# mnlevy1981/MOM6

Hardware: AMD Instinct MI355X
Metric: simulated-years/day (SYPD) of the split-RK2 dynamical core + tracer advection + ALE remap (higher is better)
Workload: dtype f64

## Files before the change

### mom6_amd/csrc/barotropic.hip

```cpp
#include "common.hpp"
#include "cr_math.hpp"

#include <algorithm>
#include <cmath>
#include <cstdlib>
#include <string>
#include <vector>

namespace {

constexpr double SUBROUNDOFF = 1e-30;

using m6::cr::cr_pow;

template <class F> __global__ void __launch_bounds__(256) range2d_kernel(int i0, int i1, int j0, int j1, F f) {
  const int i = i0 + blockIdx.x * 64 + threadIdx.x, j = j0 + blockIdx.y * 4 + threadIdx.y;
  if (i <= i1 && j <= j1) f(i, j);
}
template <class F> void launch2d(hipStream_t st, int i0, int i1, int j0, int j1, F f) {
  if (i1 < i0 || j1 < j0) return;
  dim3 grid((i1 - i0 + 64) / 64, (j1 - j0 + 4) / 4), block(64, 4);
  hipLaunchKernelGGL(range2d_kernel<F>, grid, block, 0, st, i0, i1, j0, j1, f);
}

// ... 152 lines not shown
#pragma unroll
  for (int k = 1; k < NKMAX; k++) if (k < nz) tot = tot + v[k];
  const double Ihat = mask / (tot + h_neglect);
  double *__restrict__ dst = fr + f2;
#pragma unroll
  for (int k = 0; k < NKMAX; k++) { if (k < nz) *dst = v[k] * Ihat; dst += fstr; }
}

template <int DIR>
__global__ void __launch_bounds__(256)
bt_accel_layer_kernel(m6::GridDev g, Work w, const double *__restrict__ pbce, double *__restrict__ accel, double accel_underflow) {
  const int i = (DIR ? g.isc : g.isc - 1) + blockIdx.x * 64 + threadIdx.x;
  const int j = (DIR ? g.jsc - 1 : g.jsc) + blockIdx.y * 4 + threadIdx.y;
  if (i > g.iec || j > g.jec) return;
  const long f2 = DIR ? g.v2(i, j) : g.u2(i, j);
  const long fstr = DIR ? (long)g.nih * (g.njh + 1) : (long)(g.nih + 1) * g.njh;
  const long hm = g.h2(i, j), hp = DIR ? g.h2(i, j + 1) : g.h2(i + 1, j), hstr = (long)g.nih * g.njh;
  const double abt = DIR ? w.v_accel_bt[f2] : w.u_accel_bt[f2];
  const double gp = DIR ? w.gtot_S[hp] : w.gtot_W[hp], gm = DIR ? w.gtot_N[hm] : w.gtot_E[hm];
  const double ep = w.e_anom[hp], em = w.e_anom[hm];
  const double Id = DIR ? g.IdyCv[f2] : g.IdxCu[f2];
  for (int k = 0; k < g.nk; k++) {
    double a = (abt - ((pbce[hp + hstr * k] - gp) * ep - (pbce[hm + hstr * k] - gm) * em) * Id);
    if (fabs(a) < accel_underflow) a = 0.0;
    accel[f2 + fstr * k] = a;
  }
}

__global__ void __launch_bounds__(256)
bt_eta_pred_kernel(m6::GridDev g, Work w, Par p, int i0, int i1, int j0, int j1, double wt_accel2) {
  const int i = i0 + blockIdx.x * 64 + threadIdx.x, j = j0 + blockIdx.y * 4 + threadIdx.y;
  if (i > i1 || j > j1) return;
  const long n = g.h2(i, j);
  double ep;
  if (p.project_velocity) {
    ep = w.eta[n];
  } else {
    ep = (w.eta[n] + w.eta_src[n]) + (p.dtbt * g.IareaT[n]) *
        ((w.uhbtp[g.u2(i - 1, j)] - w.uhbtp[g.u2(i, j)]) + (w.vhbtp[g.v2(i, j - 1)] - w.vhbtp[g.v2(i, j)]));
    w.eta_pred[n] = ep;
  }
  if (p.find_etaav && i >= g.isc && i <= g.iec && j >= g.jsc && j <= g.jec) w.eta_sum[n] = w.eta_sum[n] + wt_accel2 * ep;
}

__global__ void __launch_bounds__(256)
bt_eta_kernel(m6::GridDev g, Work w, Par p, int i0, int i1, int j0, int j1, double wt_eta) {
  const int i = i0 + blockIdx.x * 64 + threadIdx.x, j = j0 + blockIdx.y * 4 + threadIdx.y;
  if (i > i1 || j > j1) return;
  const long n = g.h2(i, j);
  const double e = (w.eta[n] + w.eta_src[n]) + (p.dtbt * g.IareaT[n]) *
      ((w.uhbt[g.u2(i - 1, j)] - w.uhbt[g.u2(i, j)]) + (w.vhbt[g.v2(i, j - 1)] - w.vhbt[g.v2(i, j)]));
  w.eta[n] = e;
  w.eta_wtd[n] = w.eta_wtd[n] + e * wt_eta;
}

__device__ __forceinline__ double eta_pf_at(const Work &w, const Par &p, long n, double wt_end) {
  return p.interp_eta_PF ? (w.eta_PF_1[n] + wt_end * w.d_eta_PF[n]) : w.eta_PF[n];
}

__global__ void __launch_bounds__(256)
bt_vbt_kernel(m6::GridDev g, Work w, Par p, int i0, int i1, int j0, int j1, double wt_accel, double wt_trans, double wt_end,
              double *__restrict__ vbt_sum, double *__restrict__ vhbt_sum) {
  const int i = i0 + blockIdx.x * 64 + threadIdx.x, J = j0 + blockIdx.y * 4 + threadIdx.y;
  if (i > i1 || J > j1) return;
  const int j = J;
  const long n = g.v2(i, J);
  if (w.obc_v && w.obc_v[n]) return;
  const double Cor_v = -1.0 * ((w.amer[g.u2(i - 1, j)] * w.ubt[g.u2(i - 1, j)] + w.cmer[g.u2(i, j + 1)] * w.ubt[g.u2(i, j + 1)]) +
                               (w.bmer[g.u2(i, j)] * w.ubt[g.u2(i, j)] + w.dmer[g.u2(i - 1, j + 1)] * w.ubt[g.u2(i - 1, j + 1)])) -
                       w.Cor_ref_v[n];
  const long hs = g.h2(i, j), hn = g.h2(i, j + 1);
  const double *epb = p.project_velocity ? w.eta : w.eta_pred;
  const double PFv = ((epb[hs] - eta_pf_at(w, p, hs, wt_end)) * w.gtot_N[hs] -
                      (epb[hn] - eta_pf_at(w, p, hn, wt_end)) * w.gtot_S[hn]) * p.dgeo_de * g.IdyCv[n];
  const double vel_prev = w.vbt[n];
  double vb = w.bt_rem_v[n] * (vel_prev + p.dtbt * ((w.BT_force_v[n] + Cor_v) + PFv));
  if (fabs(vb) < p.vel_underflow) vb = 0.0;
  const double vtrans = p.trans_wt1 * vb + p.trans_wt2 * vel_prev;
  w.vbt[n] = vb;
  w.v_accel_bt[n] = w.v_accel_bt[n] + wt_accel * (Cor_v + PFv);
  const double vh0 = w.vhbt0[n];
  double vh, vhp;
  if (p.use_BT_cont) { vh = find_uhbt(vtrans, w.BV, n) + vh0; vhp = find_uhbt(vb, w.BV, n) + vh0; }
  else { const double D = w.Datv[n]; vh = D * vtrans + vh0; vhp = D * vb + vh0; }
  w.vhbt[n] = vh; w.vhbtp[n] = vhp;
  if (i >= g.isc && i <= g.iec && J >= g.jsc - 1 && J <= g.jec) {
    vbt_sum[n] = vbt_sum[n] + wt_trans * vtrans;
    vhbt_sum[n] = vhbt_sum[n] + wt_trans * vh;
  }
}

__global__ void __launch_bounds__(256)
bt_ubt_kernel(m6::GridDev g, Work w, Par p, int i0, int i1, int j0, int j1, double wt_accel, double wt_trans, double wt_end,
              double *__restrict__ ubt_sum, double *__restrict__ uhbt_sum) {
  const int I = i0 + blockIdx.x * 64 + threadIdx.x, j = j0 + blockIdx.y * 4 + threadIdx.y;
  if (I > i1 || j > j1) return;
  const int i = I;
  const long n = g.u2(I, j);
  if (w.obc_u && w.obc_u[n]) return;
  const double Cor_u = ((w.azon[n] * w.vbt[g.v2(i + 1, j)] + w.czon[n] * w.vbt[g.v2(i, j - 1)]) +
                        (w.bzon[n] * w.vbt[g.v2(i, j)] + w.dzon[n] * w.vbt[g.v2(i + 1, j - 1)])) - w.Cor_ref_u[n];
  const long hw = g.h2(i, j), he = g.h2(i + 1, j);
  const double *epb = p.project_velocity ? w.eta : w.eta_pred;
  const double PFu = ((epb[hw] - eta_pf_at(w, p, hw, wt_end)) * w.gtot_E[hw] -
                      (epb[he] - eta_pf_at(w, p, he, wt_end)) * w.gtot_W[he]) * p.dgeo_de * g.IdxCu[n];
  const double vel_prev = w.ubt[n];
// ... 1032 lines not shown
  const int halo = ievf - ie, s_is = is - halo, s_ie = ie + halo, s_js = js - halo, s_je = je + halo;
  const double g_prime1 = g.g_Earth, H_to_Z = g.H_to_Z, Z_ref = cs->Z_ref;
  for (int d = 0; d < 2; d++) {
    if (!(d ? apply_v_OBCs : apply_u_OBCs)) continue;
    double *o_outer = d ? w.ob_vbt_outer : w.ob_ubt_outer, *o_dZ = d ? w.ob_dZ_v : w.ob_dZ_u,
           *o_Cg = d ? w.ob_Cg_v : w.ob_Cg_u, *o_SSH = d ? w.ob_SSH_v : w.ob_SSH_u;
    const int32_t *code = d ? w.obc_v : w.obc_u;
    launch2d(s, d ? s_is : s_is - 1, s_ie, d ? s_js - 1 : s_js, s_je, [=] __device__(int i, int j) {
      const long f = d ? g.v2(i, j) : g.u2(i, j);
      const int c = code[f];
      if (!c || (c & OB_SPEC)) return;
      {
        const long cc = (c & OB_PLUS) ? g.h2(i, j) : (d ? g.h2(i, j + 1) : g.h2(i + 1, j));
        const double dZ = g.bathyT[cc] + H_to_Z * w.eta[cc];
        o_dZ[f] = dZ;
        o_Cg[f] = sqrt(1.0 * g_prime1 * dZ);
      }
    });
    if (d ? obc->Flather_v_BCs_exist_globally : obc->Flather_u_BCs_exist_globally)
      for (int n = 0; n < obc->number_of_segments; n++) {
        const mom6hip_obc_segment_t &S = obc->segment[n];
        if (!((d ? S.is_N_or_S : S.is_E_or_W) && S.Flather)) continue;
        M6_REQUIRE(S.normal_vel_bt && S.SSH, "btstep: segment %d is a Flather segment: normal_vel_bt and SSH are required", n + 1);
        const int a0 = d ? S.isd : S.IsdB, a1 = d ? S.ied : S.IedB, b0 = d ? S.JsdB : S.jsd, b1 = d ? S.JedB : S.jed;
        const long na = a1 - a0 + 1, nb = b1 - b0 + 1;
        const double *nv = st.in(S.normal_vel_bt, (size_t)na * nb * 8), *ssh = st.in(S.SSH, (size_t)na * nb * 8);
        M6_REQUIRE(!st.failed() && nv && ssh, "btstep: staging failed");
        launch2d(s, a0, a1, b0, b1, [=] __device__(int a, int b) {
          const long f = d ? g.v2(a, b) : g.u2(a, b), q = (a - a0) + na * (b - b0);
          o_outer[f] = nv[q];
          o_SSH[f] = ssh[q] + Z_ref;
        });
      }
  }
  if (int rc = pass2d(ctx, {{w.ob_ubt_outer, PU}, {w.ob_vbt_outer, PV}, {w.ob_uhbt, PU}, {w.ob_vhbt, PV}, {w.ob_SSH_u, PUs}, {w.ob_SSH_v, PVs},
                     {w.ob_dZ_u, PUs}, {w.ob_dZ_v, PVs}, {w.ob_Cg_u, PUs}, {w.ob_Cg_v, PVs}})) return rc;
  return 0;
}

void bt_step_ranges(BtCall &bt) {
  const m6::GridDev &g = bt.g;
  const int is = g.isc, ie = g.iec, js = g.jsc, je = g.jec, isvf = bt.isvf, ievf = bt.ievf, jsvf = bt.jsvf, jevf = bt.jevf;
  const int stencil = bt.stencil, nt = bt.nt; std::vector<StepRange> &rng = bt.rng;
  rng.assign(nt + 1, StepRange{});
  int isv = is, iev = ie, jsv = js, jev = je;
  for (int n = 1; n <= nt; n++) {
    bool pf = false;
    if ((iev - stencil < ie) || (jev - stencil < je)) { pf = true; isv = isvf; iev = ievf; jsv = jsvf; jev = jevf; }
    else { isv += stencil; iev -= stencil; jsv += stencil; jev -= stencil; }
    rng[n] = {isv, iev, jsv, jev, pf};
  }
}

void bt_run_steps(BtCall &bt, hipStream_t st, int n0, int n1) {
  mom6hip_ctx_t *ctx = bt.ctx; const mom6hip_barotropic_cs_t *cs = bt.cs; const m6::GridDev &g = bt.g; const Sizes &sz = bt.sz; const Work &w = bt.w;
  const Par &p = bt.p; const CsDev &c = bt.c; const int is = g.isc, ie = g.iec, js = g.jsc, je = g.jec;
  const bool nonlin_update = bt.nonlin_update, apply_OBCs = bt.apply_OBCs, apply_u_OBCs = bt.apply_u_OBCs, apply_v_OBCs = bt.apply_v_OBCs;
  const std::vector<StepRange> &rng = bt.rng;
  const std::vector<double> &wt_vel = bt.wt_vel, &wt_eta = bt.wt_eta, &wt_trans = bt.wt_trans, &wt_accel = bt.wt_accel, &wt_accel2 = bt.wt_accel2;
  double *duhbtav = bt.duhbtav, *dvhbtav = bt.dvhbtav;
  for (int n = n0; n <= n1; n++) {
    const int isv = rng[n].isv, iev = rng[n].iev, jsv = rng[n].jsv, jev = rng[n].jev;
    const double wt_end = n * p.Instep;
    if (nonlin_update && (n > 1) && ((n - 1) % cs->Nonlin_cont_update_period == 0)) {
      find_face_areas(st, g, w.Datu, w.Datv, w.eta, 0.0, 1 + iev - ie);
      if (!p.project_velocity) {
        launch2d(st, isv - 2, iev + 1, jsv - 1, jev + 1, [=] __device__(int I, int j) {
          const long q = g.u2(I, j);
          w.uhbtp[q] = w.Datu[q] * w.ubt[q] + w.uhbt0[q];
        });
        launch2d(st, isv - 1, iev + 1, jsv - 2, jev + 1, [=] __device__(int i, int J) {
          const long q = g.v2(i, J);
          w.vhbtp[q] = w.Datv[q] * w.vbt[q] + w.vhbt0[q];
        });
      }
    }
    hipLaunchKernelGGL(bt_eta_pred_kernel, grid2d(isv - 1, iev + 1, jsv - 1, jev + 1), dim3(64, 4), 0, st, g, w, p, isv - 1, iev + 1,
                       jsv - 1, jev + 1, wt_accel2[n]);
    const bool v_first = ((n + ctx->host.first_direction) % 2) == 1;
    if (apply_OBCs) {
      (void)hipMemcpyAsync(w.ubt_old, w.ubt, sz.u2, hipMemcpyDeviceToDevice, st);
      (void)hipMemcpyAsync(w.vbt_old, w.vbt, sz.v2, hipMemcpyDeviceToDevice, st);
    }
    for (int ps = 0; ps < 2; ps++) {
      const bool do_v = (ps == 0) ? v_first : !v_first;
      if (do_v) {
        const int i0 = v_first ? isv - 1 : isv, i1 = v_first ? iev + 1 : iev;
        hipLaunchKernelGGL(bt_vbt_kernel, grid2d(i0, i1, jsv - 1, jev), dim3(64, 4), 0, st, g, w, p, i0, i1, jsv - 1, jev, wt_accel[n],
                           wt_trans[n], wt_end, c.vbtav, dvhbtav);
      } else {
        const int j0 = v_first ? jsv : jsv - 1, j1 = v_first ? jev : jev + 1;
        hipLaunchKernelGGL(bt_ubt_kernel, grid2d(isv - 1, iev, j0, j1), dim3(64, 4), 0, st, g, w, p, isv - 1, iev, j0, j1, wt_accel[n],
                           wt_trans[n], wt_end, c.ubtav, duhbtav);
      }
    }
    if (apply_OBCs) {
      const int halo = iev - ie;
      if (apply_u_OBCs)
        hipLaunchKernelGGL(bt_obc_kernel<0>, grid2d(is - halo - 1, ie + halo, js - halo, je + halo), dim3(64, 4), 0, st, g, w, p, is - halo - 1,
                           ie + halo, js - halo, je + halo, cs->bebt, wt_trans[n], wt_vel[n], c.ubtav, duhbtav);
      if (apply_v_OBCs)
        hipLaunchKernelGGL(bt_obc_kernel<1>, grid2d(is - halo, ie + halo, js - halo - 1, je + halo), dim3(64, 4), 0, st, g, w, p, is - halo,
                           ie + halo, js - halo - 1, je + halo, cs->bebt, wt_trans[n], wt_vel[n], c.vbtav, dvhbtav);
    }
    hipLaunchKernelGGL(bt_eta_kernel, grid2d(isv, iev, jsv, jev), dim3(64, 4), 0, st, g, w, p, isv, iev, jsv, jev, wt_eta[n]);
  }
}

int bt_pass_steps(BtCall &bt) {
  const Work &w = bt.w;
  return pass2d(bt.ctx, {{w.eta, PH}, {w.ubt, PU}, {w.vbt, PV}, {w.uhbtp, PU}, {w.vhbtp, PV}});
}

int bt_run_loop(BtCall &bt, hipStream_t st, int n0, int n1) {
  for (int n = n0; n <= n1; n++) {
    if (bt.rng[n].pass_first) { if (int rc = bt_pass_steps(bt)) return rc; }
    bt_run_steps(bt, st, n, n);
  }
  return 0;
}

std::string bt_graph_key(const BtCall &bt) {
  const mom6hip_barotropic_cs_t *cs = bt.cs; const CsDev &c = bt.c;
  std::string base_key;
  auto add = [&](const void *q, size_t nbytes) { base_key.append((const char *)q, nbytes); };
  add(&bt.w, sizeof(bt.w)); add(&bt.p, sizeof(bt.p)); add(&bt.nt, sizeof(bt.nt)); add(&bt.ctx->host.first_direction, sizeof(int32_t));
  { const double ob_key[3] = {bt.apply_u_OBCs ? 1.0 : 0.0, bt.apply_v_OBCs ? 1.0 : 0.0, cs->bebt}; add(ob_key, sizeof(ob_key)); }
  { const int32_t nl[2] = {bt.nonlin_update ? 1 : 0, cs->Nonlin_cont_update_period}; add(nl, sizeof(nl)); }
  add(&c.ubtav, sizeof(double *)); add(&c.vbtav, sizeof(double *)); add(&bt.duhbtav, sizeof(double *)); add(&bt.dvhbtav, sizeof(double *));
  for (const std::vector<double> *wt : {&bt.wt_vel, &bt.wt_eta, &bt.wt_trans, &bt.wt_accel, &bt.wt_accel2})
    add(wt->data(), sizeof(double) * wt->size());
  return base_key;
}

int bt_graph_of(BtCall &bt, const std::string &base_key, int n0, int n1, bool with_passes, hipGraphExec_t *out) {
  mom6hip_ctx_t *ctx = bt.ctx;
  std::string key = base_key;
  key.append((const char *)&n0, sizeof(int)); key.append((const char *)&n1, sizeof(int)); key.push_back(with_passes ? 1 : 0);
  for (auto &e : ctx->bt_graphs) if (e.first == key) { *out = (hipGraphExec_t)e.second; return 0; }
  if (!ctx->cap_stream) M6_HIP(hipStreamCreateWithFlags(&ctx->cap_stream, hipStreamNonBlocking));
  hipStream_t saved = ctx->stream;
  ctx->stream = ctx->cap_stream;
  hipError_t e0 = hipStreamBeginCapture(ctx->cap_stream, hipStreamCaptureModeRelaxed);
  int rc = 1;
  if (e0 == hipSuccess) {
    if (with_passes) rc = bt_run_loop(bt, ctx->cap_stream, n0, n1);
    else { bt_run_steps(bt, ctx->cap_stream, n0, n1); rc = 0; }
  }
  hipGraph_t graph = nullptr;
  hipError_t e1 = (e0 == hipSuccess) ? hipStreamEndCapture(ctx->cap_stream, &graph) : e0;
  ctx->stream = saved;
  M6_REQUIRE(rc == 0 && e1 == hipSuccess && graph, "btstep: capturing the barotropic subcycle as a hipGraph failed (%s)",
             hipGetErrorString(e1));
  { size_t nn = 0; if (hipGraphGetNodes(graph, nullptr, &nn) == hipSuccess) ctx->bt_graph_nodes_last = (long)nn; }
  hipGraphExec_t exec = nullptr;
  hipError_t e2 = hipGraphInstantiate(&exec, graph, nullptr, nullptr, 0);
  (void)hipGraphDestroy(graph);
  M6_REQUIRE(e2 == hipSuccess && exec, "btstep: hipGraphInstantiate failed (%s)", hipGetErrorString(e2));
  if (ctx->bt_graphs.size() >= 256) {
    (void)hipGraphExecDestroy((hipGraphExec_t)ctx->bt_graphs.front().second);
    ctx->bt_graphs.erase(ctx->bt_graphs.begin());
  }
  ctx->bt_graphs.push_back({key, (void *)exec});
  ctx->bt_graph_captures++;
  *out = exec;
  return 0;
}

int bt_segments(const BtCall &bt) {
  int nseg = 0;
  for (int n = 1; n <= bt.nt; n++) if (n == 1 || bt.rng[n].pass_first) nseg++;
  return nseg;
}

int bt_subcycle(BtCall &bt) {
  mom6hip_ctx_t *ctx = bt.ctx; hipStream_t s = bt.s; const int nt = bt.nt; const std::vector<StepRange> &rng = bt.rng;
  static const bool graph_off = getenv("MOM6HIP_BT_GRAPH") && atoi(getenv("MOM6HIP_BT_GRAPH")) == 0;
  if (graph_off || (m6::multi_tile(ctx) && bt_segments(bt) > 100)) {
    if (int rc = bt_run_loop(bt, s, 1, nt)) return rc;
  } else if (m6::multi_tile(ctx)) {
    const std::string base_key = bt_graph_key(bt);
    int n0 = 1;
    while (n0 <= nt) {
      int n1 = n0;
      while (n1 + 1 <= nt && !rng[n1 + 1].pass_first) n1++;
      if (rng[n0].pass_first) { if (int rc = bt_pass_steps(bt)) return rc; }
      hipGraphExec_t exec = nullptr;
      if (int rc = bt_graph_of(bt, base_key, n0, n1, false, &exec)) return rc;
      M6_HIP(hipGraphLaunch(exec, s));
      ctx->bt_graph_launches++;
      n0 = n1 + 1;
    }
  } else {
    hipGraphExec_t exec = nullptr;
    if (int rc = bt_graph_of(bt, bt_graph_key(bt), 1, nt, true, &exec)) return rc;
    m6::KTimer kt(ctx, MOM6HIP_KT_BT_SUBCYCLE);
    M6_HIP(hipGraphLaunch(exec, s));
    ctx->bt_graph_launches++;
  }
  M6_HIP(hipGetLastError());
  return 0;
}

int bt_epilogue(BtCall &bt) {
  mom6hip_ctx_t *ctx = bt.ctx; const m6::GridDev &g = bt.g; const Work &w = bt.w; const Par &p = bt.p; const CsDev &c = bt.c; hipStream_t s = bt.s;
  const int is = g.isc, ie = g.iec, js = g.jsc, je = g.jec;
  const bool interp = bt.interp, find_etaav = bt.find_etaav, apply_OBCs = bt.apply_OBCs, apply_u_OBCs = bt.apply_u_OBCs,
             apply_v_OBCs = bt.apply_v_OBCs;
  const double dt = bt.dt, accel_underflow = bt.accel_underflow; const double *deta_in = bt.deta_in, *dpb = bt.dpb;
  double *dalu = bt.dalu, *dalv = bt.dalv, *deta_out = bt.deta_out, *duhbtav = bt.duhbtav, *dvhbtav = bt.dvhbtav, *detaav = bt.detaav;
  const double dgeo_de = p.dgeo_de;
  launch2d(s, is, ie, js, je, [=] __device__(int i, int j) {
    const long n = g.h2(i, j);
    double ea;
    if (interp) ea = dgeo_de * (0.5 * (w.eta[n] + deta_in[n]) - (w.eta_PF_1[n] + 0.5 * w.d_eta_PF[n]));
    else ea = dgeo_de * (0.5 * (w.eta[n] + deta_in[n]) - w.eta_PF[n]);
    w.e_anom[n] = ea;
    if (find_etaav) detaav[n] = w.eta_sum[n] * 1.0;
    deta_out[n] = w.eta_wtd[n] * 1.0;
  });
  for (int d = 0; d < 2 && apply_OBCs; d++) {
    if (!(d ? apply_v_OBCs : apply_u_OBCs)) continue;
    const int32_t *code = d ? w.obc_v : w.obc_u;
    launch2d(s, d ? is : is - 1, ie, d ? js - 1 : js, je, [=] __device__(int i, int j) {
      const int cde = code[d ? g.v2(i, j) : g.u2(i, j)];
      const long c0 = g.h2(i, j), c1 = d ? g.h2(i, j + 1) : g.h2(i + 1, j);
      if (cde & OB_PLUS) w.e_anom[c1] = w.e_anom[c0];
      else if (cde & OB_MINUS) w.e_anom[c0] = w.e_anom[c1];
    });
  }
  if (find_etaav) { if (int rc = pass2d(ctx, {{detaav, PH}, {w.e_anom, PH}, {c.ubtav, PU}, {c.vbtav, PV}, {duhbtav, PU}, {dvhbtav, PV}})) return rc; }
  else { if (int rc = pass2d(ctx, {{w.e_anom, PH}, {c.ubtav, PU}, {c.vbtav, PV}, {duhbtav, PU}, {dvhbtav, PV}})) return rc; }
  hipLaunchKernelGGL(bt_accel_layer_kernel<0>, grid2d(is - 1, ie, js, je), dim3(64, 4), 0, s, g, w, dpb, dalu, accel_underflow);
  hipLaunchKernelGGL(bt_accel_layer_kernel<1>, grid2d(is, ie, js - 1, je), dim3(64, 4), 0, s, g, w, dpb, dalv, accel_underflow);
  for (int d = 0; d < 2 && apply_OBCs; d++) {
    if (!(d ? apply_v_OBCs : apply_u_OBCs)) continue;
    const int32_t *code = d ? w.obc_v : w.obc_u;
    const double *wtd = d ? w.vbt_wtd : w.ubt_wtd, *first = d ? w.vbt_first : w.ubt_first;
// ... 70 lines not shown
```

### mom6_amd/csrc/context.hip

```cpp
#include <cstdarg>
#include <cmath>

#include <cstring>

#include "common.hpp"

#include <vector>

namespace m6 {

static thread_local std::string g_err;

void set_error(const char *fmt, ...) {
  char buf[1024];
  va_list ap;
  va_start(ap, fmt);
  vsnprintf(buf, sizeof(buf), fmt, ap);
  va_end(ap);
  g_err = buf;
}
ErrorKeeper::ErrorKeeper() { snprintf(saved, sizeof(saved), "%s", g_err.c_str()); }
ErrorKeeper::~ErrorKeeper() { g_err = saved; }

int DevBuf::reserve(size_t n) {
// ... 333 lines not shown
    double *d = nullptr;
    rc = upload2d(ctx, un.data(), nU, &d); g.uh_neglect = d;
    if (!rc) { rc = upload2d(ctx, vn.data(), nV, &d); g.vh_neglect = d; }
    if (!rc && hipStreamSynchronize(ctx->stream) != hipSuccess) { set_error("grid upload failed"); rc = 1; }
    if (rc) { mom6hip_grid_destroy(ctx); return rc; }
  }
  if (hipHostMalloc((void **)&ctx->h_domore_k, sizeof(int) * (size_t)(grid->nk + 1), hipHostMallocDefault) != hipSuccess) {
    set_error("hipHostMalloc failed"); mom6hip_grid_destroy(ctx); return 1;
  }
  *out = ctx;
  return 0;
}

int mom6hip_grid_destroy(mom6hip_ctx_t *ctx) {
  if (!ctx) return 0;
  (void)hipStreamSynchronize(ctx->stream);
  m6::native_domain_destroy(ctx);
  for (void *p : ctx->metric_allocs) (void)hipFree(p);
  ctx->hprev.release(); ctx->uhr.release(); ctx->vhr.release(); ctx->flags.release();
  for (auto &b : ctx->stage) b.release();
  for (auto &b : ctx->tr_stage) b.release();
  for (auto &b : ctx->pool) b.release();
  ctx->rk2_scratch.release(); ctx->rk2_eta_PF_start.release(); ctx->cont_hmid.release();
  for (auto &e : ctx->obc_tables) e.buf.release();
  for (auto &t : ctx->tables) t.buf.release();
  ctx->hv_pack.release(); ctx->hv_str.release();
  ctx->ale_sub.release();
  ctx->ale_side.release();
  ctx->vv_ntrunc.release(); ctx->vv_kvml[0].release(); ctx->vv_kvml[1].release();
  ctx->efp_acc.release();
  for (auto &e : ctx->bt_graphs) (void)hipGraphExecDestroy((hipGraphExec_t)e.second);
  if (ctx->cap_stream) (void)hipStreamDestroy(ctx->cap_stream);
  for (hipStream_t st : ctx->side_stream) if (st) (void)hipStreamDestroy(st);
  if (ctx->side_fork) (void)hipEventDestroy(ctx->side_fork);
  for (hipEvent_t e : ctx->side_join) if (e) (void)hipEventDestroy(e);
  m6::staging_destroy(ctx);
  if (ctx->h_domore_k) (void)hipHostFree(ctx->h_domore_k);
  delete ctx;
  return 0;
}

}

namespace {

struct HaloDesc {
  double *f;
  int ilo, jlo;
  int nis, njs, nk;
  int ics, ice, jcs, jce, ni, nj, ihi, jhi;
  int poison;
};

__global__ void halo_x_kernel(HaloDesc d) {
  const int nwl = d.ics - d.ilo, nwr = d.ihi - d.ice;
  const int nw = nwl + nwr;
  const long total = (long)nw * (d.jce - d.jcs + 1) * d.nk;
  for (long t = blockIdx.x * (long)blockDim.x + threadIdx.x; t < total; t += (long)gridDim.x * blockDim.x) {
    int h = (int)(t % nw);
    long r = t / nw;
    int j = d.jcs + (int)(r % (d.jce - d.jcs + 1));
    int k = (int)(r / (d.jce - d.jcs + 1));
    int i, src;
    if (h < nwl) { i = d.ilo + h; src = i + d.ni; } else { i = d.ice + 1 + (h - nwl); src = i - d.ni; }
    long base = (long)d.nis * ((long)(j - d.jlo) + (long)d.njs * k);
    if (d.poison) { if (d.poison & (h < nwl ? 1 : 2)) d.f[base + (i - d.ilo)] = __builtin_nan(""); continue; }
    d.f[base + (i - d.ilo)] = d.f[base + (src - d.ilo)];
  }
}

__global__ void halo_y_kernel(HaloDesc d) {
  const int nws = d.jcs - d.jlo, nwn = d.jhi - d.jce;
  const int nw = nws + nwn;
  const long total = (long)d.nis * nw * d.nk;
  for (long t = blockIdx.x * (long)blockDim.x + threadIdx.x; t < total; t += (long)gridDim.x * blockDim.x) {
    int ii = (int)(t % d.nis);
    long r = t / d.nis;
    int h = (int)(r % nw);
    int k = (int)(r / nw);
    int j, src;
    if (h < nws) { j = d.jlo + h; src = j + d.nj; } else { j = d.jce + 1 + (h - nws); src = j - d.nj; }
    long kb = (long)d.nis * d.njs * k;
    if (d.poison) { if (d.poison & (h < nws ? 1 : 2)) d.f[kb + (long)d.nis * (j - d.jlo) + ii] = __builtin_nan(""); continue; }
    d.f[kb + (long)d.nis * (j - d.jlo) + ii] = d.f[kb + (long)d.nis * (src - d.jlo) + ii];
  }
}

__global__ void halo_fold_kernel(HaloDesc d, int isum, int ys, int negate) {
  const int nwn = d.jhi - d.jce;
  const long total = (long)d.nis * nwn * d.nk;
  for (long t = blockIdx.x * (long)blockDim.x + threadIdx.x; t < total; t += (long)gridDim.x * blockDim.x) {
    const int ii = (int)(t % d.nis);
    long r = t / d.nis;
    const int m = 1 + (int)(r % nwn);
    const int k = (int)(r / nwn);
    const int si = isum - (d.ilo + ii);
    if (si < d.ilo || si > d.ihi) continue;
    const int j = d.jce + m, sj = ys ? d.jce - m : d.jce + 1 - m;
    const long kb = (long)d.nis * d.njs * k;
    const double v = d.poison ? __builtin_nan("") : d.f[kb + (long)d.nis * (sj - d.jlo) + (si - d.ilo)];
    d.f[kb + (long)d.nis * (j - d.jlo) + ii] = negate ? -v : v;
  }
}

}

namespace m6 {

int halo_fold_north(mom6hip_ctx_t *ctx, double *f, int pos_flags, int nk, hipStream_t stream) {
  const mom6hip_grid_t &G = ctx->host;
  const int pos = pos_flags & 3;
  const int xs = (pos == MOM6HIP_POS_U || pos == MOM6HIP_POS_Q) ? 1 : 0;
  const int ys = (pos == MOM6HIP_POS_V || pos == MOM6HIP_POS_Q) ? 1 : 0;
  const int negate = ((pos == MOM6HIP_POS_U || pos == MOM6HIP_POS_V) && !(pos_flags & MOM6HIP_PASS_SCALAR_PAIR)) ? 1 : 0;
  HaloDesc d;
  d.f = f; d.ilo = G.isd - xs; d.jlo = G.jsd - ys; d.ihi = G.ied; d.jhi = G.jed;
  d.nis = d.ihi - d.ilo + 1; d.njs = d.jhi - d.jlo + 1; d.nk = nk;
  d.ics = G.isc - xs; d.ice = G.iec; d.jcs = G.jsc - ys; d.jce = G.jec;
  d.ni = G.iec - G.isc + 1; d.nj = G.jec - G.jsc + 1; d.poison = ctx->poison_now;
  const long total = (long)d.nis * (d.jhi - d.jce) * nk;
  if (total > 0) {
    int blocks = (int)((total + 255) / 256); if (blocks > 4096) blocks = 4096;
    hipLaunchKernelGGL(halo_fold_kernel, dim3(blocks), dim3(256), 0, stream, d, G.isc + G.iec - xs, ys, negate);
  }
  M6_HIP(hipGetLastError());
  return 0;
}

int halo_wrap_dir(mom6hip_ctx_t *ctx, double *f, int pos_flags, int nk, int dir, hipStream_t stream) {
  const mom6hip_grid_t &G = ctx->host;
  const int pos = pos_flags & 3;
  const int xs = (pos == MOM6HIP_POS_U || pos == MOM6HIP_POS_Q) ? 1 : 0;
  const int ys = (pos == MOM6HIP_POS_V || pos == MOM6HIP_POS_Q) ? 1 : 0;
  HaloDesc d;
  d.f = f; d.ilo = G.isd - xs; d.jlo = G.jsd - ys; d.ihi = G.ied; d.jhi = G.jed;
  d.nis = d.ihi - d.ilo + 1; d.njs = d.jhi - d.jlo + 1; d.nk = nk;
  d.ics = G.isc - xs; d.ice = G.iec; d.jcs = G.jsc - ys; d.jce = G.jec;
  d.ni = G.iec - G.isc + 1; d.nj = G.jec - G.jsc + 1; d.poison = ctx->poison_now;
  if (dir == 0) {
    long total = (long)((d.ics - d.ilo) + (d.ihi - d.ice)) * (d.jce - d.jcs + 1) * nk;
    if (total > 0) {
      int blocks = (int)((total + 255) / 256); if (blocks > 4096) blocks = 4096;
      hipLaunchKernelGGL(halo_x_kernel, dim3(blocks), dim3(256), 0, stream, d);
    }
  } else {
    long total = (long)d.nis * ((d.jcs - d.jlo) + (d.jhi - d.jce)) * nk;
    if (total > 0) {
      int blocks = (int)((total + 255) / 256); if (blocks > 4096) blocks = 4096;
      hipLaunchKernelGGL(halo_y_kernel, dim3(blocks), dim3(256), 0, stream, d);
    }
  }
  M6_HIP(hipGetLastError());
  return 0;
}

int halo_update_field(mom6hip_ctx_t *ctx, double *f, int pos, int nk) {
  const mom6hip_grid_t &G = ctx->host;
  if (G.reentrant_x) if (int rc = halo_wrap_dir(ctx, f, pos, nk, 0, ctx->stream)) return rc;
  if (G.reentrant_y) if (int rc = halo_wrap_dir(ctx, f, pos, nk, 1, ctx->stream)) return rc;
  if (G.tripolar_n) if (int rc = halo_fold_north(ctx, f, pos, nk, ctx->stream)) return rc;
  return 0;
}

namespace {
int start_now(mom6hip_ctx_t *ctx, double *const *fields, const int32_t *pos, const int32_t *nk, int n) {
  if (ctx->native) return native_start_group_pass(ctx, fields, pos, nk, n);
  if (ctx->halo_cb) {
    if (!ctx->cb_stream_ordered) M6_HIP(hipStreamSynchronize(ctx->stream));
    M6_REQUIRE(ctx->halo_cb(ctx->cb_user, fields, pos, nk, n) == 0, "group pass: the domain halo callback failed");
    return 0;
  }
  for (int f = 0; f < n; f++)
    if (int rc = halo_update_field(ctx, fields[f], pos[f], nk[f])) return rc;
  return 0;
}
}

int start_group_pass(mom6hip_ctx_t *ctx, double *const *fields, const int32_t *pos, const int32_t *nk, int n) {
  if (!ctx->poison_passes) return start_now(ctx, fields, pos, nk, n);
  M6_REQUIRE(ctx->pending.f.empty(), "start_group_pass: a pass is already in flight");
  M6_REQUIRE(!ctx->halo_cb || ctx->native, "mom6hip_debug_poison_passes: not provided for the host's halo callback");
  const mom6hip_grid_t &G = ctx->host;
  int sides[2] = {0, G.reentrant_y ? 3 : 0};
  if (ctx->native) native_pass_sides(ctx, sides);
  if (G.reentrant_x && (!ctx->native || native_x_is_local(ctx)))
    for (int f = 0; f < n; f++)
      if (int rc = halo_wrap_dir(ctx, fields[f], pos[f], nk[f], 0, ctx->stream)) return rc;
  for (int f = 0; f < n; f++) {
    for (int dir = 0; dir < 2; dir++) {
      if (!sides[dir]) continue;
      ctx->poison_now = sides[dir];
      const int rc = halo_wrap_dir(ctx, fields[f], pos[f], nk[f], dir, ctx->stream);
      ctx->poison_now = 0;
      if (rc) return rc;
    }
    if (G.tripolar_n) {
      ctx->poison_now = 3;
      const int rc = halo_fold_north(ctx, fields[f], pos[f], nk[f], ctx->stream);
      ctx->poison_now = 0;
      if (rc) return rc;
    }
  }
  ctx->pending.f.assign(fields, fields + n); ctx->pending.pos.assign(pos, pos + n); ctx->pending.nk.assign(nk, nk + n);
  return 0;
}

int complete_group_pass(mom6hip_ctx_t *ctx) {
  if (ctx->poison_passes && !ctx->pending.f.empty()) {
    auto &P = ctx->pending;
    const int rc = start_now(ctx, P.f.data(), P.pos.data(), P.nk.data(), (int)P.f.size());
    P.f.clear(); P.pos.clear(); P.nk.clear();
    if (rc) return rc;
  }
  if (ctx->native) return native_complete_group_pass(ctx);
  return 0;
}

int group_pass(mom6hip_ctx_t *ctx, double *const *fields, const int32_t *pos, const int32_t *nk, int n) {
  if (int rc = start_group_pass(ctx, fields, pos, nk, n)) return rc;
  return complete_group_pass(ctx);
}

bool pass_leaves_x_final(mom6hip_ctx_t *ctx) { return ctx->native ? native_x_is_local(ctx) : (ctx->halo_cb == nullptr); }
void row_window(mom6hip_ctx_t *ctx, int j0, int j1) { ctx->g.jsc = j0; ctx->g.jec = j1; }
void row_window_reset(mom6hip_ctx_t *ctx) { ctx->g.jsc = ctx->host.jsc; ctx->g.jec = ctx->host.jec; }

int sum_across_PEs(mom6hip_ctx_t *ctx, int32_t *values, int n) {
  if (ctx->native) return native_allreduce(ctx, values, n, true);
  if (ctx->sum_cb) M6_REQUIRE(ctx->sum_cb(ctx->cb_user, values, n) == 0, "the host's sum_across_PEs failed");
  return 0;
}

int sum_across_PEs_dev(mom6hip_ctx_t *ctx, int32_t *dvalues, int n, int32_t *host_copy) {
  if (ctx->native) return native_allreduce_dev(ctx, dvalues, n, 0, host_copy);
  std::vector<int32_t> tmp;
  int32_t *h = host_copy;
  if (!h) { tmp.resize((size_t)n); h = tmp.data(); }
  M6_HIP(hipMemcpyAsync(h, dvalues, sizeof(int32_t) * (size_t)n, hipMemcpyDeviceToHost, ctx->stream));
  M6_HIP(hipStreamSynchronize(ctx->stream));
  if (!ctx->sum_cb) return 0;
// ... 132 lines not shown
```

Before: 26.88.

## Fuse barotropic eta update with next step's predictor and batch halo wraps

The barotropic loop now runs whole stretches of steps between halo passes in one call. Within a stretch, each step's eta update kernel also computes the next step's eta predictor over the inner range, so one launch and one re-read of eta and the fluxes per substep are dropped. Separately, periodic halo wraps for a group of fields are batched into one launch per direction (up to eight fields, one per grid.y slot), replacing one launch per field. The costs are extra range checks, a graph key that now hashes the step ranges, and reliance on the next predictor range lying inside the current update range.

Result: no change. 26.98, median of 2 (+0.4%).

```diff
diff --git a/mom6_amd/csrc/barotropic.hip b/mom6_amd/csrc/barotropic.hip
--- a/mom6_amd/csrc/barotropic.hip
+++ b/mom6_amd/csrc/barotropic.hip
@@ -228,6 +228,28 @@
       ((w.uhbt[g.u2(i - 1, j)] - w.uhbt[g.u2(i, j)]) + (w.vhbt[g.v2(i, j - 1)] - w.vhbt[g.v2(i, j)]));
   w.eta[n] = e;
   w.eta_wtd[n] = w.eta_wtd[n] + e * wt_eta;
+}
+
+__global__ void __launch_bounds__(256)
+bt_eta_pair_kernel(m6::GridDev g, Work w, Par p, int i0, int i1, int j0, int j1, double wt_eta, int pi0, int pi1, int pj0, int pj1,
+                   double wt_accel2) {
+  const int i = i0 + blockIdx.x * 64 + threadIdx.x, j = j0 + blockIdx.y * 4 + threadIdx.y;
+  if (i > i1 || j > j1) return;
+  const long n = g.h2(i, j);
+  const long uw = g.u2(i - 1, j), ue = g.u2(i, j), vs = g.v2(i, j - 1), vn = g.v2(i, j);
+  const double src = w.eta_src[n], dtA = p.dtbt * g.IareaT[n];
+  const double e = (w.eta[n] + src) + dtA * ((w.uhbt[uw] - w.uhbt[ue]) + (w.vhbt[vs] - w.vhbt[vn]));
+  w.eta[n] = e;
+  w.eta_wtd[n] = w.eta_wtd[n] + e * wt_eta;
+  if (i < pi0 || i > pi1 || j < pj0 || j > pj1) return;
+  double ep;
+  if (p.project_velocity) {
+    ep = e;
+  } else {
+    ep = (e + src) + dtA * ((w.uhbtp[uw] - w.uhbtp[ue]) + (w.vhbtp[vs] - w.vhbtp[vn]));
+    w.eta_pred[n] = ep;
+  }
+  if (p.find_etaav && i >= g.isc && i <= g.iec && j >= g.jsc && j <= g.jec) w.eta_sum[n] = w.eta_sum[n] + wt_accel2 * ep;
 }
 
 __device__ __forceinline__ double eta_pf_at(const Work &w, const Par &p, long n, double wt_end) {
@@ -1366,17 +1388,24 @@
   }
 }
 
-void bt_run_steps(BtCall &bt, hipStream_t st, int n0, int n1) {
+bool bt_refresh_first(const BtCall &bt, int n) {
+  return bt.nonlin_update && (n > 1) && ((n - 1) % bt.cs->Nonlin_cont_update_period == 0);
+}
+bool bt_pairs_with_next(const BtCall &bt, int n) {
+  return (n < bt.nt) && !bt.rng[n + 1].pass_first && !bt_refresh_first(bt, n + 1);
+}
+
+int bt_run_steps(BtCall &bt, hipStream_t st, int n0, int n1) {
   mom6hip_ctx_t *ctx = bt.ctx; const mom6hip_barotropic_cs_t *cs = bt.cs; const m6::GridDev &g = bt.g; const Sizes &sz = bt.sz; const Work &w = bt.w;
   const Par &p = bt.p; const CsDev &c = bt.c; const int is = g.isc, ie = g.iec, js = g.jsc, je = g.jec;
-  const bool nonlin_update = bt.nonlin_update, apply_OBCs = bt.apply_OBCs, apply_u_OBCs = bt.apply_u_OBCs, apply_v_OBCs = bt.apply_v_OBCs;
+  const bool apply_OBCs = bt.apply_OBCs, apply_u_OBCs = bt.apply_u_OBCs, apply_v_OBCs = bt.apply_v_OBCs;
   const std::vector<StepRange> &rng = bt.rng;
   const std::vector<double> &wt_vel = bt.wt_vel, &wt_eta = bt.wt_eta, &wt_trans = bt.wt_trans, &wt_accel = bt.wt_accel, &wt_accel2 = bt.wt_accel2;
   double *duhbtav = bt.duhbtav, *dvhbtav = bt.dvhbtav;
   for (int n = n0; n <= n1; n++) {
     const int isv = rng[n].isv, iev = rng[n].iev, jsv = rng[n].jsv, jev = rng[n].jev;
     const double wt_end = n * p.Instep;
-    if (nonlin_update && (n > 1) && ((n - 1) % cs->Nonlin_cont_update_period == 0)) {
+    if (bt_refresh_first(bt, n)) {
       find_face_areas(st, g, w.Datu, w.Datv, w.eta, 0.0, 1 + iev - ie);
       if (!p.project_velocity) {
         launch2d(st, isv - 2, iev + 1, jsv - 1, jev + 1, [=] __device__(int I, int j) {
@@ -1389,8 +1418,9 @@
         });
       }
     }
-    hipLaunchKernelGGL(bt_eta_pred_kernel, grid2d(isv - 1, iev + 1, jsv - 1, jev + 1), dim3(64, 4), 0, st, g, w, p, isv - 1, iev + 1,
-                       jsv - 1, jev + 1, wt_accel2[n]);
+    if (!(n > n0 && bt_pairs_with_next(bt, n - 1)))
+      hipLaunchKernelGGL(bt_eta_pred_kernel, grid2d(isv - 1, iev + 1, jsv - 1, jev + 1), dim3(64, 4), 0, st, g, w, p, isv - 1, iev + 1,
+                         jsv - 1, jev + 1, wt_accel2[n]);
     const bool v_first = ((n + ctx->host.first_direction) % 2) == 1;
     if (apply_OBCs) {
       (void)hipMemcpyAsync(w.ubt_old, w.ubt, sz.u2, hipMemcpyDeviceToDevice, st);
@@ -1417,8 +1447,18 @@
         hipLaunchKernelGGL(bt_obc_kernel<1>, grid2d(is - halo, ie + halo, js - halo - 1, je + halo), dim3(64, 4), 0, st, g, w, p, is - halo,
                            ie + halo, js - halo - 1, je + halo, cs->bebt, wt_trans[n], wt_vel[n], c.vbtav, dvhbtav);
     }
-    hipLaunchKernelGGL(bt_eta_kernel, grid2d(isv, iev, jsv, jev), dim3(64, 4), 0, st, g, w, p, isv, iev, jsv, jev, wt_eta[n]);
-  }
+    if (n < n1 && bt_pairs_with_next(bt, n)) {
+      const int pi0 = rng[n + 1].isv - 1, pi1 = rng[n + 1].iev + 1, pj0 = rng[n + 1].jsv - 1, pj1 = rng[n + 1].jev + 1;
+      M6_REQUIRE(pi0 >= isv && pi1 <= iev && pj0 >= jsv && pj1 <= jev,
+                 "btstep: the predictor range of step %d (%d..%d, %d..%d) is not inside the range of step %d (%d..%d, %d..%d)", n + 1, pi0,
+                 pi1, pj0, pj1, n, isv, iev, jsv, jev);
+      hipLaunchKernelGGL(bt_eta_pair_kernel, grid2d(isv, iev, jsv, jev), dim3(64, 4), 0, st, g, w, p, isv, iev, jsv, jev, wt_eta[n], pi0,
+                         pi1, pj0, pj1, wt_accel2[n + 1]);
+    } else {
+      hipLaunchKernelGGL(bt_eta_kernel, grid2d(isv, iev, jsv, jev), dim3(64, 4), 0, st, g, w, p, isv, iev, jsv, jev, wt_eta[n]);
+    }
+  }
+  return 0;
 }
 
 int bt_pass_steps(BtCall &bt) {
@@ -1426,10 +1466,18 @@
   return pass2d(bt.ctx, {{w.eta, PH}, {w.ubt, PU}, {w.vbt, PV}, {w.uhbtp, PU}, {w.vhbtp, PV}});
 }
 
+int bt_stretch_end(const BtCall &bt, int n0, int n1) {
+  int n = n0;
+  while (n + 1 <= n1 && !bt.rng[n + 1].pass_first) n++;
+  return n;
+}
+
 int bt_run_loop(BtCall &bt, hipStream_t st, int n0, int n1) {
-  for (int n = n0; n <= n1; n++) {
-    if (bt.rng[n].pass_first) { if (int rc = bt_pass_steps(bt)) return rc; }
-    bt_run_steps(bt, st, n, n);
+  for (int a = n0; a <= n1;) {
+    const int b = bt_stretch_end(bt, a, n1);
+    if (bt.rng[a].pass_first) { if (int rc = bt_pass_steps(bt)) return rc; }
+    if (int rc = bt_run_steps(bt, st, a, b)) return rc;
+    a = b + 1;
   }
   return 0;
 }
@@ -1444,6 +1492,11 @@
   add(&c.ubtav, sizeof(double *)); add(&c.vbtav, sizeof(double *)); add(&bt.duhbtav, sizeof(double *)); add(&bt.dvhbtav, sizeof(double *));
   for (const std::vector<double> *wt : {&bt.wt_vel, &bt.wt_eta, &bt.wt_trans, &bt.wt_accel, &bt.wt_accel2})
     add(wt->data(), sizeof(double) * wt->size());
+  for (int n = 1; n <= bt.nt; n++) {
+    const StepRange &r = bt.rng[n];
+    const int32_t rk[5] = {r.isv, r.iev, r.jsv, r.jev, r.pass_first ? 1 : 0};
+    add(rk, sizeof(rk));
+  }
   return base_key;
 }
 
@@ -1459,7 +1512,7 @@
   int rc = 1;
   if (e0 == hipSuccess) {
     if (with_passes) rc = bt_run_loop(bt, ctx->cap_stream, n0, n1);
-    else { bt_run_steps(bt, ctx->cap_stream, n0, n1); rc = 0; }
+    else rc = bt_run_steps(bt, ctx->cap_stream, n0, n1);
   }
   hipGraph_t graph = nullptr;
   hipError_t e1 = (e0 == hipSuccess) ? hipStreamEndCapture(ctx->cap_stream, &graph) : e0;
@@ -1496,8 +1549,7 @@
     const std::string base_key = bt_graph_key(bt);
     int n0 = 1;
     while (n0 <= nt) {
-      int n1 = n0;
-      while (n1 + 1 <= nt && !rng[n1 + 1].pass_first) n1++;
+      const int n1 = bt_stretch_end(bt, n0, nt);
       if (rng[n0].pass_first) { if (int rc = bt_pass_steps(bt)) return rc; }
       hipGraphExec_t exec = nullptr;
       if (int rc = bt_graph_of(bt, base_key, n0, n1, false, &exec)) return rc;
diff --git a/mom6_amd/csrc/context.hip b/mom6_amd/csrc/context.hip
--- a/mom6_amd/csrc/context.hip
+++ b/mom6_amd/csrc/context.hip
@@ -409,7 +409,10 @@
   int poison;
 };
 
-__global__ void halo_x_kernel(HaloDesc d) {
+constexpr int HALO_BATCH = 8;
+struct HaloBatch { HaloDesc d[HALO_BATCH]; };
+
+__device__ __forceinline__ void halo_x_wrap(const HaloDesc &d) {
   const int nwl = d.ics - d.ilo, nwr = d.ihi - d.ice;
   const int nw = nwl + nwr;
   const long total = (long)nw * (d.jce - d.jcs + 1) * d.nk;
@@ -425,8 +428,10 @@
     d.f[base + (i - d.ilo)] = d.f[base + (src - d.ilo)];
   }
 }
-
-__global__ void halo_y_kernel(HaloDesc d) {
+__global__ void halo_x_kernel(HaloDesc d) { halo_x_wrap(d); }
+__global__ void halo_x_batch_kernel(HaloBatch b) { halo_x_wrap(b.d[blockIdx.y]); }
+
+__device__ __forceinline__ void halo_y_wrap(const HaloDesc &d) {
   const int nws = d.jcs - d.jlo, nwn = d.jhi - d.jce;
   const int nw = nws + nwn;
   const long total = (long)d.nis * nw * d.nk;
@@ -442,6 +447,8 @@
     d.f[kb + (long)d.nis * (j - d.jlo) + ii] = d.f[kb + (long)d.nis * (src - d.jlo) + ii];
   }
 }
+__global__ void halo_y_kernel(HaloDesc d) { halo_y_wrap(d); }
+__global__ void halo_y_batch_kernel(HaloBatch b) { halo_y_wrap(b.d[blockIdx.y]); }
 
 __global__ void halo_fold_kernel(HaloDesc d, int isum, int ys, int negate) {
   const int nwn = d.jhi - d.jce;
@@ -460,31 +467,7 @@
   }
 }
 
-}
-
-namespace m6 {
-
-int halo_fold_north(mom6hip_ctx_t *ctx, double *f, int pos_flags, int nk, hipStream_t stream) {
-  const mom6hip_grid_t &G = ctx->host;
-  const int pos = pos_flags & 3;
-  const int xs = (pos == MOM6HIP_POS_U || pos == MOM6HIP_POS_Q) ? 1 : 0;
-  const int ys = (pos == MOM6HIP_POS_V || pos == MOM6HIP_POS_Q) ? 1 : 0;
-  const int negate = ((pos == MOM6HIP_POS_U || pos == MOM6HIP_POS_V) && !(pos_flags & MOM6HIP_PASS_SCALAR_PAIR)) ? 1 : 0;
-  HaloDesc d;
-  d.f = f; d.ilo = G.isd - xs; d.jlo = G.jsd - ys; d.ihi = G.ied; d.jhi = G.jed;
-  d.nis = d.ihi - d.ilo + 1; d.njs = d.jhi - d.jlo + 1; d.nk = nk;
-  d.ics = G.isc - xs; d.ice = G.iec; d.jcs = G.jsc - ys; d.jce = G.jec;
-  d.ni = G.iec - G.isc + 1; d.nj = G.jec - G.jsc + 1; d.poison = ctx->poison_now;
-  const long total = (long)d.nis * (d.jhi - d.jce) * nk;
-  if (total > 0) {
-    int blocks = (int)((total + 255) / 256); if (blocks > 4096) blocks = 4096;
-    hipLaunchKernelGGL(halo_fold_kernel, dim3(blocks), dim3(256), 0, stream, d, G.isc + G.iec - xs, ys, negate);
-  }
-  M6_HIP(hipGetLastError());
-  return 0;
-}
-
-int halo_wrap_dir(mom6hip_ctx_t *ctx, double *f, int pos_flags, int nk, int dir, hipStream_t stream) {
+HaloDesc halo_desc_of(const mom6hip_ctx_t *ctx, double *f, int pos_flags, int nk) {
   const mom6hip_grid_t &G = ctx->host;
   const int pos = pos_flags & 3;
   const int xs = (pos == MOM6HIP_POS_U || pos == MOM6HIP_POS_Q) ? 1 : 0;
@@ -494,18 +477,61 @@
   d.nis = d.ihi - d.ilo + 1; d.njs = d.jhi - d.jlo + 1; d.nk = nk;
   d.ics = G.isc - xs; d.ice = G.iec; d.jcs = G.jsc - ys; d.jce = G.jec;
   d.ni = G.iec - G.isc + 1; d.nj = G.jec - G.jsc + 1; d.poison = ctx->poison_now;
-  if (dir == 0) {
-    long total = (long)((d.ics - d.ilo) + (d.ihi - d.ice)) * (d.jce - d.jcs + 1) * nk;
-    if (total > 0) {
-      int blocks = (int)((total + 255) / 256); if (blocks > 4096) blocks = 4096;
-      hipLaunchKernelGGL(halo_x_kernel, dim3(blocks), dim3(256), 0, stream, d);
+  return d;
+}
+long halo_wrap_total(const HaloDesc &d, int dir) {
+  return dir == 0 ? (long)((d.ics - d.ilo) + (d.ihi - d.ice)) * (d.jce - d.jcs + 1) * d.nk
+                  : (long)d.nis * ((d.jcs - d.jlo) + (d.jhi - d.jce)) * d.nk;
+}
+int halo_blocks(long total) { const long b = (total + 255) / 256; return (int)(b > 4096 ? 4096 : b); }
+
+}
+
+namespace m6 {
+
+int halo_fold_north(mom6hip_ctx_t *ctx, double *f, int pos_flags, int nk, hipStream_t stream) {
+  const mom6hip_grid_t &G = ctx->host;
+  const int pos = pos_flags & 3;
+  const int xs = (pos == MOM6HIP_POS_U || pos == MOM6HIP_POS_Q) ? 1 : 0;
+  const int ys = (pos == MOM6HIP_POS_V || pos == MOM6HIP_POS_Q) ? 1 : 0;
+  const int negate = ((pos == MOM6HIP_POS_U || pos == MOM6HIP_POS_V) && !(pos_flags & MOM6HIP_PASS_SCALAR_PAIR)) ? 1 : 0;
+  const HaloDesc d = halo_desc_of(ctx, f, pos_flags, nk);
+  const long total = (long)d.nis * (d.jhi - d.jce) * nk;
+  if (total > 0) {
+    hipLaunchKernelGGL(halo_fold_kernel, dim3(halo_blocks(total)), dim3(256), 0, stream, d, G.isc + G.iec - xs, ys, negate);
+  }
+  M6_HIP(hipGetLastError());
+  return 0;
+}
+
+int halo_wrap_dir(mom6hip_ctx_t *ctx, double *f, int pos_flags, int nk, int dir, hipStream_t stream) {
+  const HaloDesc d = halo_desc_of(ctx, f, pos_flags, nk);
+  const long total = halo_wrap_total(d, dir);
+  if (total > 0) {
+    if (dir == 0) hipLaunchKernelGGL(halo_x_kernel, dim3(halo_blocks(total)), dim3(256), 0, stream, d);
+    else hipLaunchKernelGGL(halo_y_kernel, dim3(halo_blocks(total)), dim3(256), 0, stream, d);
+  }
+  M6_HIP(hipGetLastError());
+  return 0;
+}
+
+int halo_wrap_dir_all(mom6hip_ctx_t *ctx, double *const *fields, const int32_t *pos, const int32_t *nk, int n, int dir,
+                      hipStream_t stream) {
+  M6_REQUIRE(ctx->poison_now == 0, "halo_wrap_dir_all: not for the poisoning of a pass");
+  for (int f0 = 0; f0 < n; f0 += HALO_BATCH) {
+    HaloBatch b;
+    int nb = 0; long most = 0;
+    for (int f = f0; f < n && f < f0 + HALO_BATCH; f++) {
+      const HaloDesc d = halo_desc_of(ctx, fields[f], pos[f], nk[f]);
+      const long total = halo_wrap_total(d, dir);
+      if (total <= 0) continue;
+      b.d[nb++] = d;
+      if (total > most) most = total;
     }
-  } else {
-    long total = (long)d.nis * ((d.jcs - d.jlo) + (d.jhi - d.jce)) * nk;
-    if (total > 0) {
-      int blocks = (int)((total + 255) / 256); if (blocks > 4096) blocks = 4096;
-      hipLaunchKernelGGL(halo_y_kernel, dim3(blocks), dim3(256), 0, stream, d);
-    }
+    if (nb == 0) continue;
+    for (int q = nb; q < HALO_BATCH; q++) b.d[q] = b.d[0];
+    if (dir == 0) hipLaunchKernelGGL(halo_x_batch_kernel, dim3(halo_blocks(most), nb), dim3(256), 0, stream, b);
+    else hipLaunchKernelGGL(halo_y_batch_kernel, dim3(halo_blocks(most), nb), dim3(256), 0, stream, b);
   }
   M6_HIP(hipGetLastError());
   return 0;
@@ -527,8 +553,12 @@
     M6_REQUIRE(ctx->halo_cb(ctx->cb_user, fields, pos, nk, n) == 0, "group pass: the domain halo callback failed");
     return 0;
   }
-  for (int f = 0; f < n; f++)
-    if (int rc = halo_update_field(ctx, fields[f], pos[f], nk[f])) return rc;
+  const mom6hip_grid_t &G = ctx->host;
+  if (G.reentrant_x) if (int rc = halo_wrap_dir_all(ctx, fields, pos, nk, n, 0, ctx->stream)) return rc;
+  if (G.reentrant_y) if (int rc = halo_wrap_dir_all(ctx, fields, pos, nk, n, 1, ctx->stream)) return rc;
+  if (G.tripolar_n)
+    for (int f = 0; f < n; f++)
+      if (int rc = halo_fold_north(ctx, fields[f], pos[f], nk[f], ctx->stream)) return rc;
   return 0;
 }
 }
@@ -541,8 +571,7 @@
   int sides[2] = {0, G.reentrant_y ? 3 : 0};
   if (ctx->native) native_pass_sides(ctx, sides);
   if (G.reentrant_x && (!ctx->native || native_x_is_local(ctx)))
-    for (int f = 0; f < n; f++)
-      if (int rc = halo_wrap_dir(ctx, fields[f], pos[f], nk[f], 0, ctx->stream)) return rc;
+    if (int rc = halo_wrap_dir_all(ctx, fields, pos, nk, n, 0, ctx->stream)) return rc;
   for (int f = 0; f < n; f++) {
     for (int dir = 0; dir < 2; dir++) {
       if (!sides[dir]) continue;
```
